# DrorT/demucs

Measured on NVIDIA B200. Metric: htdemucs audio-seconds separated per second, higher is better.
Workload: dtype f32 (bf16 hi/lo split operands, 3 tcgen05 products, fp32 accumulate)

## Files before the change

### demucs_b200/csrc/gemm_tc_impl.cuh

```cuda
#pragma once
#include <stdlib.h>
#include "gemm_epilogue.cuh"
#include "tcgen05.cuh"

enum { BD_TC_TF32 = 0, BD_TC_TF32X3 = 1, BD_TC_BF16X3 = 2, BD_TC_BF16 = 3, BD_TC_BF16D = 4 };

struct TileGeom {
  int R0, R1;
  int log2R0;
  int blocks0, blocks1;
  int cpb;
  int stride4;
};

namespace {

constexpr int TBM = 128;


struct RowInfo {
  long long obase;
  int i0;
  int rb_row;
  float e_mean, e_rstd;
  int pad0, pad1;
};

__device__ __forceinline__ float sigmoid_fast(float x) {
  const float e = bd_ex2_approx(-1.44269504088896340736f * x);
  float r;
  asm("rcp.approx.ftz.f32 %0, %1;" : "=f"(r) : "f"(1.0f + e));
  return r;
}
__device__ __forceinline__ float4 lds128(uint32_t a) {
  float4 v;
  asm volatile("ld.shared.v4.f32 {%0, %1, %2, %3}, [%4];" : "=f"(v.x), "=f"(v.y), "=f"(v.z), "=f"(v.w) : "r"(a));
  return v;
}

template <int ACT, bool E, bool RES, bool ROWB, bool CT, int WC, int RB>
__device__ __forceinline__ void epi_fast_rows(const bd_gemm_desc& d, uint32_t stage_s, uint32_t rinfo_s, int lane, int n0w,
                                              float& ssum, float& ssq) {
  constexpr int LDT = WC + 4;
  constexpr int CG = WC / 4 < 32 ? WC / 4 : 32;
  constexpr int RPI = 32 / CG;
  const int cg = lane % CG, rsub = lane / CG;
  const int n = n0w + 4 * cg;
  const bool col_ok = n < d.N;
  const int nc = col_ok ? n : 0;
  const float4 bias = d.bias ? ldg4(d.bias + nc) : make_float4(0.f, 0.f, 0.f, 0.f);
  float4 gam = make_float4(1.f, 1.f, 1.f, 1.f), bet = make_float4(0.f, 0.f, 0.f, 0.f);
  if (E) {
    gam = ldg4(d.e_gamma + nc);
    bet = ldg4(d.e_beta + nc);
  }
  const int no = ACT == BD_ACT_GLU ? nc >> 1 : nc;
  float4 scl = make_float4(1.f, 1.f, 1.f, 1.f);
  if (RES && d.scale) {
    if (ACT == BD_ACT_GLU) {
      const float2 t = ldg2(d.scale + no);
      scl.x = t.x; scl.y = t.y;
    } else {
      scl = ldg4(d.scale + no);
    }
  }
  int rr = 0;
  long long colofs = no;
  if (CT) {
    const int cout = d.N >> 2;
    rr = nc / cout;
    colofs = (long long)rr * d.os_0 + (nc - rr * cout);
    rr -= d.convt == 1 ? 2 : 0;
  }
  const long long outo = colofs;
  const float* resp = RES ? d.resid + colofs : nullptr;
  const float* addp = CT && d.addend ? d.addend + colofs : nullptr;
  const float* rbp = ROWB ? d.rowbias + no : nullptr;
  const int rb_ld = ACT == BD_ACT_GLU ? d.N >> 1 : d.N;
  const uint32_t st_lane = stage_s + (uint32_t)(rsub * LDT + 4 * cg) * 4u;
  const uint32_t ri_lane = rinfo_s + (uint32_t)rsub * 32u;
#pragma unroll 1
  for (int it = 0; it < 32 / RPI; it += RB) {
    long long ob[RB];
    bool ok[RB];
    float mean[RB], rstd[RB];
    float4 res[RB];
#pragma unroll
    for (int u = 0; u < RB; ++u) {
      const uint32_t ra = ri_lane + (uint32_t)((it + u) * RPI) * 32u;
      uint32_t w0, w1, w2, w3;
      asm volatile("ld.shared.v4.u32 {%0, %1, %2, %3}, [%4];" : "=r"(w0), "=r"(w1), "=r"(w2), "=r"(w3) : "r"(ra));
      ob[u] = (long long)(((unsigned long long)w1 << 32) | w0);
      ok[u] = (int)w2 >= 0 && col_ok;
      if (CT) ok[u] = ok[u] && (unsigned)(4 * (int)w2 + rr) < (unsigned)d.O0;
      if (ROWB || CT) res[u] = make_float4(0.f, 0.f, 0.f, 0.f);
      if (ROWB && ok[u]) {
        if (ACT == BD_ACT_GLU) {
          const float2 t = ldg2(rbp + (size_t)w3 * rb_ld);
          res[u].x = t.x; res[u].y = t.y;
        } else {
          res[u] = ldg4(rbp + (size_t)w3 * rb_ld);
        }
      }
      if (CT && addp && ok[u]) res[u] = ldg4(addp + ob[u]);
      if (E) asm volatile("ld.shared.v2.f32 {%0, %1}, [%2];" : "=f"(mean[u]), "=f"(rstd[u]) : "r"(ra + 16));
      if (RES) {
        res[u] = make_float4(0.f, 0.f, 0.f, 0.f);
        if (ok[u]) {
          if (ACT == BD_ACT_GLU) {
            const float2 t = ldg2(resp + ob[u]);
            res[u].x = t.x; res[u].y = t.y;
          } else {
            res[u] = ldg4(resp + ob[u]);
          }
        }
      }
    }
#pragma unroll
    for (int u = 0; u < RB; ++u) {
      float4 v = lds128(st_lane + (uint32_t)((it + u) * RPI * LDT) * 4u);
      v.x += bias.x; v.y += bias.y; v.z += bias.z; v.w += bias.w;
      if (E) {
        v.x = fmaf((v.x - mean[u]) * rstd[u], gam.x, bet.x);
        v.y = fmaf((v.y - mean[u]) * rstd[u], gam.y, bet.y);
        v.z = fmaf((v.z - mean[u]) * rstd[u], gam.z, bet.z);
        v.w = fmaf((v.w - mean[u]) * rstd[u], gam.w, bet.w);
      }
      if (ACT == BD_ACT_GLU) {
        float2 o2 = make_float2(v.x * sigmoid_fast(v.y), v.z * sigmoid_fast(v.w));
        if (ROWB) {
          o2.x += res[u].x;
          o2.y += res[u].y;
        }
        if (RES) {
          o2.x = fmaf(scl.x, o2.x, res[u].x);
          o2.y = fmaf(scl.y, o2.y, res[u].y);
        }
        if (ok[u]) {
          bd_store_out2(d, outo + ob[u], o2);
          ssum += o2.x + o2.y;
          ssq = fmaf(o2.x, o2.x, fmaf(o2.y, o2.y, ssq));
        }
      } else {
        if (ACT == BD_ACT_GELU) {
          v.x = bd_gelu(v.x); v.y = bd_gelu(v.y); v.z = bd_gelu(v.z); v.w = bd_gelu(v.w);
        }
        if (RES) {
          v.x = fmaf(scl.x, v.x, res[u].x); v.y = fmaf(scl.y, v.y, res[u].y);
          v.z = fmaf(scl.z, v.z, res[u].z); v.w = fmaf(scl.w, v.w, res[u].w);
        }
        if (ROWB || CT) {
          v.x += res[u].x; v.y += res[u].y; v.z += res[u].z; v.w += res[u].w;
        }
        if (ok[u]) {
          bd_store_out4(d, outo + ob[u], v);
          ssum += (v.x + v.y) + (v.z + v.w);
          ssq = fmaf(v.x, v.x, fmaf(v.y, v.y, fmaf(v.z, v.z, fmaf(v.w, v.w, ssq))));
        }
      }
    }
  }
}

__device__ __forceinline__ int epi_fast_id(const bd_gemm_desc& d, bool vec, bool row_stats) {
  if (!vec || row_stats || !d.out || d.oc_split) return -1;
  const bool e = d.e_stats != nullptr, r = d.resid != nullptr;
  if (d.convt) return (d.act == BD_ACT_GELU && !e && !r && !d.rowbias) ? 6 : -1;
  if (d.addend) return -1;
  if (d.rowbias) return (d.act == BD_ACT_GLU && !e && !r) ? 5 : -1;
  if (d.act == BD_ACT_NONE && !e) return r ? 1 : 0;
  if (d.act == BD_ACT_GELU && !e && !r) return 2;
  if (d.act == BD_ACT_GLU && !e && !r) return 3;
  if (d.act == BD_ACT_GLU && e && r) return 4;
  return -1;
}

#ifndef BD_TC_EPI_GROUPS
#define BD_TC_EPI_GROUPS 4
#endif
__host__ __device__ constexpr int pow2_at_least(int v, int p) { return p >= v ? p : pow2_at_least(v, 2 * p); }

template <int TBK, int TBN, int MODE, bool ATM = false>
struct PCfg {
  static_assert(!ATM || (MODE == BD_TC_BF16X3 && TBN <= 192), "A in tensor memory: strict mode, tiles up to 192 wide");
  static_assert(TBN % 16 == 0 && TBN <= 256, "UMMA N (M = 128): a multiple of 16 up to 256");
  static constexpr bool kX3 = MODE == BD_TC_TF32X3;
  static constexpr bool kB16 = MODE == BD_TC_BF16X3 || MODE == BD_TC_BF16 || MODE == BD_TC_BF16D;
  static constexpr bool kDirect = MODE == BD_TC_BF16D;
  static constexpr bool kSplit = MODE != BD_TC_TF32 && !kDirect;
  static constexpr int kBParts = MODE == BD_TC_BF16X3 ? 2 : 1;
  static constexpr int kPGroups = (MODE == BD_TC_TF32X3 || MODE == BD_TC_BF16X3) ? 2 : BD_TC_EPI_GROUPS;
  static constexpr int kSplitWarp0 = kB16 ? 2 : 4;
  static constexpr int kSplitWarps = MODE == BD_TC_BF16 ? 2 : 4;
  static constexpr int kEpiWarp0 = kSplit ? kSplitWarp0 + kSplitWarps : 4;
  static constexpr int kThreads = 32 * kEpiWarp0 + 128 * kPGroups;
  static constexpr int kTileBytesA = TBM * TBK * (kDirect ? 2 : 4);
  static constexpr int kTileBytesB = kB16 ? TBN * TBK * 2 : TBN * TBK * 4;
  static constexpr int kStageBytesA = (kX3 ? 2 : 1) * kTileBytesA;
  static constexpr int kStageBytesB = (kX3 ? 2 : kBParts) * kTileBytesB;
  static constexpr int kTxBytes = kTileBytesA + (kB16 ? kBParts : 1) * kTileBytesB;
  static constexpr bool kTileSplit = TBN <= 32;
  static constexpr int kNAcc = kTileSplit ? kPGroups : 2;
  static constexpr int kChunk = TBN == 256 ? 128 : TBN == 192 ? 64 : TBN == 96 ? 32 : TBN;
  static constexpr int kChunks = TBN / kChunk;
  static constexpr int kWarpCols = kTileSplit ? TBN : kChunk / kPGroups;
  static_assert(kWarpCols >= 16 && (kWarpCols & (kWarpCols - 1)) == 0, "epilogue: power-of-two warp column range");
  static constexpr int kStagingBytes = 4 * kPGroups * 32 * (kWarpCols + 4) * 4;
  static constexpr int kTailBytes = 512 + 128 * kPGroups * 32;
  static constexpr int kBudget = 227 * 1024 - 1024 - kTailBytes - kStagingBytes;
  static constexpr int kStagesRaw = kBudget / (kStageBytesA + kStageBytesB);
  static constexpr int kStages = kStagesRaw > (kTileSplit ? 16 : 8) ? (kTileSplit ? 16 : 8) : kStagesRaw;
  static constexpr int kSmemBytes = kStages * (kStageBytesA + kStageBytesB) + kStagingBytes + 1024 + kTailBytes;
  static constexpr int kACol0 = kNAcc * TBN;
  static constexpr int kTmemUsed = kNAcc * TBN + (ATM ? kStages * TBK : 0);
  static_assert(kTmemUsed <= 512, "tensor memory: accumulators + A ring exceed 512 columns");
  static constexpr int kTmemCols = pow2_at_least(kTmemUsed, 32);
};

template <int TBK, int TBN, int MODE, bool ATM>
__global__ void __launch_bounds__((PCfg<TBK, TBN, MODE, ATM>::kThreads), 1) conv_gemm_tc_persist_kernel(const __grid_constant__ CUtensorMap map_a,
                                                                            const __grid_constant__ CUtensorMap map_b,
                                                                            const __grid_constant__ CUtensorMap map_b_lo,
                                                                            const bd_gemm_desc d, const TileGeom g,
                                                                            int ntiles, int ntn) {
  using C_ = PCfg<TBK, TBN, MODE, ATM>;
  constexpr bool X3 = C_::kX3, B16 = C_::kB16, SPLIT = C_::kSplit;
  constexpr int kPGroups = C_::kPGroups;
  constexpr int kTileBytesA = C_::kTileBytesA, kTileBytesB = C_::kTileBytesB;
  constexpr int kStages = C_::kStages, kStageBytesA = C_::kStageBytesA, kStageBytesB = C_::kStageBytesB;
  constexpr int kTmemCols = C_::kTmemCols;
  constexpr int WC = C_::kWarpCols;
  constexpr int CW = WC < 32 ? WC : 32;
  extern __shared__ uint8_t smem_raw[];
  uint8_t* smem = reinterpret_cast<uint8_t*>(((uintptr_t)smem_raw + 1023) & ~(uintptr_t)1023);
  uint8_t* sA = smem;
  uint8_t* sB = smem + kStages * kStageBytesA;
  float* staging = reinterpret_cast<float*>(sB + kStages * kStageBytesB);
  uint64_t* full_bar = reinterpret_cast<uint64_t*>(reinterpret_cast<uint8_t*>(staging) + C_::kStagingBytes);
  uint64_t* empty_bar = full_bar + kStages;
  constexpr int kNAcc = C_::kNAcc;
  constexpr bool kTileSplit = C_::kTileSplit;
  constexpr int NCH = C_::kChunks, CHW = C_::kChunk;
  uint64_t* tmem_full = empty_bar + kStages;
  uint64_t* tmem_empty = tmem_full + kNAcc;
  uint64_t* conv_bar = tmem_empty + kNAcc;
  uint32_t* tmem_slot = reinterpret_cast<uint32_t*>(conv_bar + kStages);

  const int warp = threadIdx.x >> 5, lane = threadIdx.x & 31;
  const int nkb = d.taps * g.cpb;

  if (threadIdx.x == 0) {
    for (int s = 0; s < kStages; ++s) {
      mbar_init(&full_bar[s], 1);
      mbar_init(&empty_bar[s], 1);
      mbar_init(&conv_bar[s], 32 * C_::kSplitWarps);
    }
    for (int a = 0; a < kNAcc; ++a) {
      mbar_init(&tmem_full[a], 1);
      mbar_init(&tmem_empty[a], kTileSplit ? 4 : 4 * kPGroups);
    }
    mbar_fence_init();
  }
  if (warp == 1) {
    tcgen05_alloc(tmem_slot, kTmemCols);
    tcgen05_relinquish();
  }
  tcgen05_fence_before();
  __syncthreads();
  tcgen05_fence_after();
  const uint32_t tmem_base = *tmem_slot;

  auto decode = [&](int tile, int& b, int& i0s, int& i1s, int& n0) {
    const int nb = tile % ntn;
    int r = tile / ntn;
    const int blk0 = r % g.blocks0;
    r /= g.blocks0;
    const int blk1 = r % g.blocks1;
    b = r / g.blocks1;
    i0s = blk0 * g.R0;
    i1s = blk1 * g.R1;
    n0 = nb * TBN;
  };

  if (warp == 0) {
    if (lane == 0) {
      long long kbg = 0;
      for (int tile = blockIdx.x; tile < ntiles; tile += gridDim.x) {
        int b, i0s, i1s, n0;
        decode(tile, b, i0s, i1s, n0);
        int tap = 0, cb = 0;
        for (int kb = 0; kb < nkb; ++kb, ++kbg) {
          const int s = (int)(kbg % kStages);
          const uint32_t ph = (uint32_t)((kbg / kStages) & 1);
          mbar_wait_parked(&empty_bar[s], ph ^ 1);
          mbar_expect_tx(&full_bar[s], C_::kTxBytes);
          if (g.stride4) {
            const int d0 = d.d0[tap];
            tma_load_5d(&map_a, &full_bar[s], sA + s * kStageBytesA, cb * TBK, d0 & 3, i0s + (d0 >> 2), i1s + d.d1[tap], b);
          } else {
            tma_load_4d(&map_a, &full_bar[s], sA + s * kStageBytesA, cb * TBK, i0s + d.d0[tap], i1s + d.d1[tap], b);
          }
          tma_load_2d(&map_b, &full_bar[s], sB + s * kStageBytesB, tap * d.Cin + cb * TBK, n0);
          if constexpr (MODE == BD_TC_BF16X3)
            tma_load_2d(&map_b_lo, &full_bar[s], sB + s * kStageBytesB + kTileBytesB, tap * d.Cin + cb * TBK, n0);
          if (++cb == g.cpb) {
            cb = 0;
            ++tap;
// ... 99 lines not shown
      constexpr int RB = TBK * 4, RH = TBK * 2;
      constexpr int GB = 8 * RB;
      constexpr int SW = C_::kSplitWarps;
      constexpr int NG = (TBM / 8) / SW;
      const int sw = warp - C_::kSplitWarp0, r = lane >> 2, q = lane & 3;
      const int xin = (r * RB >> 7) & (RB / 16 - 1);
      const int xout = (r * RH >> 7) & (RH / 16 - 1);
      (void)et;
      for (int tile = blockIdx.x; tile < ntiles; tile += gridDim.x) {
        for (int kb = 0; kb < nkb; ++kb, ++kbg) {
          const int s = (int)(kbg % kStages);
          mbar_wait(&full_bar[s], (uint32_t)((kbg / kStages) & 1));
          uint8_t* base = sA + s * kStageBytesA;
#pragma unroll
          for (int i0 = 0; i0 < NG; i0 += 4) {
          float4 v[4][TBK == 32 ? 2 : 1];
#pragma unroll
          for (int i = 0; i < 4; ++i) {
            const uint8_t* gp = base + (sw + SW * (i0 + i)) * GB + r * RB;
            if constexpr (TBK == 32) {
              v[i][0] = *reinterpret_cast<const float4*>(gp + (((2 * q) ^ xin) << 4));
              v[i][1] = *reinterpret_cast<const float4*>(gp + (((2 * q + 1) ^ xin) << 4));
            } else {
              v[i][0] = *reinterpret_cast<const float4*>(gp + ((q ^ xin) << 4));
            }
          }
          __syncwarp();
#pragma unroll
          for (int i = 0; i < 4; ++i) {
            uint8_t* gp = base + (sw + SW * (i0 + i)) * GB + r * RH;
            uint32_t hi[TBK == 32 ? 4 : 2], lo[TBK == 32 ? 4 : 2];
#pragma unroll
            for (int j = 0; j < (TBK == 32 ? 2 : 1); ++j) {
              const float4 x = v[i][j];
              const uint32_t h0 = bd_pack_bf16(x.x, x.y), h1 = bd_pack_bf16(x.z, x.w);
              hi[2 * j] = h0;
              hi[2 * j + 1] = h1;
              lo[2 * j] = lo[2 * j + 1] = 0u;
              if constexpr (MODE == BD_TC_BF16X3) {
                lo[2 * j] = bd_pack_bf16(x.x - __uint_as_float(h0 << 16), x.y - __uint_as_float(h0 & 0xffff0000u));
                lo[2 * j + 1] = bd_pack_bf16(x.z - __uint_as_float(h1 << 16), x.w - __uint_as_float(h1 & 0xffff0000u));
              }
            }
            if constexpr (TBK == 32) {
              uint8_t* dst = gp + ((q ^ xout) << 4);
              *reinterpret_cast<uint4*>(dst) = make_uint4(hi[0], hi[1], hi[2], hi[3]);
              if constexpr (MODE == BD_TC_BF16X3) *reinterpret_cast<uint4*>(dst + 8 * RH) = make_uint4(lo[0], lo[1], lo[2], lo[3]);
            } else {
              uint8_t* dst = gp + (((q >> 1) ^ xout) << 4) + ((q & 1) << 3);
              *reinterpret_cast<uint2*>(dst) = make_uint2(hi[0], hi[1]);
              if constexpr (MODE == BD_TC_BF16X3) *reinterpret_cast<uint2*>(dst + 8 * RH) = make_uint2(lo[0], lo[1]);
            }
          }
          }
          asm volatile("fence.proxy.async.shared::cta;" ::: "memory");
          mbar_arrive(&conv_bar[s]);
        }
      }
    } else {
    for (int tile = blockIdx.x; tile < ntiles; tile += gridDim.x) {
      for (int kb = 0; kb < nkb; ++kb, ++kbg) {
        const int s = (int)(kbg % kStages);
        mbar_wait(&full_bar[s], (uint32_t)((kbg / kStages) & 1));
        auto split = [&](uint8_t* base, int tile_bytes) {
          float4* hi = reinterpret_cast<float4*>(base);
          float4* lo = reinterpret_cast<float4*>(base + tile_bytes);
#pragma unroll 4
          for (int i = et; i < tile_bytes / 16; i += 128) {
            const float4 x = hi[i];
            const float4 h = make_float4(bd_tf32_rna(x.x), bd_tf32_rna(x.y), bd_tf32_rna(x.z), bd_tf32_rna(x.w));
            hi[i] = h;
            lo[i] = make_float4(x.x - h.x, x.y - h.y, x.z - h.z, x.w - h.w);
          }
        };
        split(sA + s * kStageBytesA, kTileBytesA);
        split(sB + s * kStageBytesB, kTileBytesB);
        asm volatile("fence.proxy.async.shared::cta;" ::: "memory");
        mbar_arrive(&conv_bar[s]);
      }
    }
    }
  } else if (warp >= C_::kEpiWarp0) {
    const int quarter = warp & 3, ew = warp - C_::kEpiWarp0, grp = ew >> 2;
    const int cbase = kTileSplit ? 0 : grp * WC;
    const bool row_stats = d.stats_out && d.stat_mod != 1;
    const bool vec = bd_epi_vec_ok(d);
    const int fast = epi_fast_id(d, vec, row_stats);
    constexpr int LDT = WC + 4;
    float* stage = staging + (size_t)ew * 32 * LDT;
    RowInfo* rinfo = reinterpret_cast<RowInfo*>(((uintptr_t)(tmem_slot + 4) + 31) & ~(uintptr_t)31) + ew * 32;
    int tcount = 0;
    for (int tile = blockIdx.x; tile < ntiles; tile += gridDim.x, ++tcount) {
      if (kTileSplit && tcount % kPGroups != grp) continue;
      int b, i0s, i1s, n0;
      decode(tile, b, i0s, i1s, n0);
      const int a = tcount % kNAcc;
      const int r = quarter * 32 + lane;
      const int i0 = i0s + (r & (g.R0 - 1)), i1 = i1s + (r >> g.log2R0);
      const bool row_ok = i0 < d.I0 && i1 < d.I1;
      const long long m = ((long long)b * d.I1 + i1) * d.I0 + i0;
      EpiRow er;
      er.obase = 0; er.i0 = 0; er.rb_row = 0; er.e_mean = 0.f; er.e_rstd = 1.f;
      if (row_ok) {
        er.i0 = i0;
        er.obase = (long long)b * d.os_b + (long long)i1 * d.os_1 +
                   (long long)(d.convt ? 4 * i0 - (d.convt == 1 ? 2 : 0) : i0) * d.os_0;
        if (d.rowbias) er.rb_row = (int)((unsigned)m % (unsigned)d.rowbias_period);
        if (d.e_stats) {
          const int sl = bd_stat_slab(d, m);
          er.e_mean = __ldg(d.e_stats + 2 * (size_t)sl);
          er.e_rstd = __ldg(d.e_stats + 2 * (size_t)sl + 1);
        }
      }
      const int my_slab = (d.stats_out && row_ok) ? bd_stat_slab(d, m) : -1;
      float ssum = 0.f, ssq = 0.f;
      if (d.resid && row_ok && !d.convt && !d.oc_split) {
        const int c0 = n0 + cbase;
        if (c0 < d.N) {
          const float* pf = d.resid + er.obase + (d.act == BD_ACT_GLU ? c0 >> 1 : c0);
          asm volatile("prefetch.global.L2 [%0];" ::"l"(pf));
        }
      }
#pragma unroll 1
      for (int ch = 0; ch < NCH; ++ch) {
      const int n0h = n0 + CHW * ch;
      if (ch == 0) {
        mbar_wait_relaxed(&tmem_full[a], (uint32_t)((tcount / kNAcc) & 1));
        tcgen05_fence_after();
      } else {
        __syncwarp();
      }
      const bool last_chunk = ch == NCH - 1;
      const uint32_t acc = tmem_base + (uint32_t)(a * TBN + CHW * ch + cbase) + ((uint32_t)(quarter * 32) << 16);
      if (vec) {
        rinfo[lane].obase = er.obase;
        rinfo[lane].i0 = row_ok ? er.i0 : -1;
        rinfo[lane].rb_row = er.rb_row;
        rinfo[lane].e_mean = er.e_mean;
        rinfo[lane].e_rstd = er.e_rstd;
        for (int c0 = 0; c0 < WC; c0 += CW) {
          if (n0h + cbase + c0 >= d.N) break;
          uint32_t v[CW];
          if constexpr (CW == 32) tmem_ld32(acc + c0, v); else tmem_ld16(acc + c0, v);
#pragma unroll
          for (int j = 0; j < CW; j += 4)
            *reinterpret_cast<float4*>(stage + lane * LDT + c0 + j) =
                make_float4(__uint_as_float(v[j]), __uint_as_float(v[j + 1]), __uint_as_float(v[j + 2]),
                            __uint_as_float(v[j + 3]));
        }
        tcgen05_fence_before();
        __syncwarp();
        if (lane == 0 && last_chunk) mbar_arrive(&tmem_empty[a]);
        if (fast >= 0) {
          const uint32_t st_s = smem_u32(stage), ri_s = smem_u32(rinfo);
          const int n0w = n0h + cbase;
          constexpr int FRB = kPGroups >= 4 ? 2 : 4;
          switch (fast) {
            case 0: epi_fast_rows<BD_ACT_NONE, false, false, false, false, WC, FRB>(d, st_s, ri_s, lane, n0w, ssum, ssq); break;
            case 1: epi_fast_rows<BD_ACT_NONE, false, true, false, false, WC, FRB>(d, st_s, ri_s, lane, n0w, ssum, ssq); break;
            case 2: epi_fast_rows<BD_ACT_GELU, false, false, false, false, WC, FRB>(d, st_s, ri_s, lane, n0w, ssum, ssq); break;
            case 3: epi_fast_rows<BD_ACT_GLU, false, false, false, false, WC, FRB>(d, st_s, ri_s, lane, n0w, ssum, ssq); break;
            case 4: epi_fast_rows<BD_ACT_GLU, true, true, false, false, WC, FRB>(d, st_s, ri_s, lane, n0w, ssum, ssq); break;
            case 5: epi_fast_rows<BD_ACT_GLU, false, false, true, false, WC, FRB>(d, st_s, ri_s, lane, n0w, ssum, ssq); break;
            default: epi_fast_rows<BD_ACT_GELU, false, false, false, true, WC, FRB>(d, st_s, ri_s, lane, n0w, ssum, ssq); break;
          }
          __syncwarp();
        } else {
        constexpr int CG = WC / 4 < 32 ? WC / 4 : 32;
        constexpr int RPI = 32 / CG;
        constexpr int RB = kPGroups >= 4 ? 2 : 4;
        const int cg = lane % CG, rsub = lane / CG;
        const int n = n0h + cbase + 4 * cg;
        const bool col_ok = n < d.N;
        EpiCol ecol;
        if (col_ok) ecol = bd_epi_cols4(d, n);
        for (int it = 0; it < 32 / RPI; it += RB) {
          EpiRow row[RB];
          EpiMem mem[RB];
          bool ok[RB];
#pragma unroll
          for (int u = 0; u < RB; ++u) {
            const int rloc = (it + u) * RPI + rsub;
            const uint32_t ra = smem_u32(&rinfo[rloc]);
            uint32_t w0, w1, w2, w3, w4, w5;
            asm volatile("ld.shared.v4.u32 {%0, %1, %2, %3}, [%4];" : "=r"(w0), "=r"(w1), "=r"(w2), "=r"(w3) : "r"(ra));
            asm volatile("ld.shared.v2.u32 {%0, %1}, [%2];" : "=r"(w4), "=r"(w5) : "r"(ra + 16));
            row[u].obase = (long long)(((unsigned long long)w1 << 32) | w0);
            row[u].i0 = (int)w2;
            row[u].rb_row = (int)w3;
            row[u].e_mean = __uint_as_float(w4);
            row[u].e_rstd = __uint_as_float(w5);
            ok[u] = row[u].i0 >= 0 && col_ok;
            if (ok[u]) mem[u] = bd_epi_fetch4(d, row[u], ecol);
          }
#pragma unroll
          for (int u = 0; u < RB; ++u) {
            const int rloc = (it + u) * RPI + rsub;
            float rs = 0.f, rq = 0.f;
            if (ok[u]) {
              const float4 acc4 = *reinterpret_cast<const float4*>(stage + rloc * LDT + 4 * cg);
              bd_epi_finish4(d, row[u], ecol, acc4, mem[u], rs, rq);
            }
            if (row_stats) {
              __syncwarp();
              *reinterpret_cast<float2*>(stage + rloc * LDT + 2 * cg) = make_float2(rs, rq);
            } else {
              ssum += rs;
              ssq += rq;
            }
          }
        }
        if (row_stats) {
          __syncwarp();
          float rs = 0.f, rq = 0.f;
#pragma unroll
          for (int c = 0; c < CG; ++c) {
            const float2 t = *reinterpret_cast<const float2*>(stage + lane * LDT + 2 * c);
            rs += t.x;
            rq += t.y;
          }
          if (my_slab >= 0) {
            atomicAdd(&d.stats_out[2 * (size_t)my_slab], (double)rs);
            atomicAdd(&d.stats_out[2 * (size_t)my_slab + 1], (double)rq);
          }
        }
        __syncwarp();
        }
      } else {
        for (int c0 = 0; c0 < WC; c0 += CW) {
          if (n0h + cbase + c0 >= d.N) break;
          uint32_t v[CW];
          if constexpr (CW == 32) tmem_ld32(acc + c0, v); else tmem_ld16(acc + c0, v);
          if (row_ok) {
#pragma unroll
            for (int j = 0; j < CW; ++j) {
              const int n = n0h + cbase + c0 + j;
              if (n < d.N) {
                float st;
                if (bd_epi_apply(d, er, n, __uint_as_float(v[j]), __uint_as_float(v[(j + 1) % CW]), st)) {
                  ssum += st;
                  ssq = fmaf(st, st, ssq);
                }
              }
            }
          }
        }
        tcgen05_fence_before();
        __syncwarp();
        if (lane == 0 && last_chunk) mbar_arrive(&tmem_empty[a]);
      }
      }
      if (!vec && row_stats && row_ok) {
        atomicAdd(&d.stats_out[2 * (size_t)my_slab], (double)ssum);
        atomicAdd(&d.stats_out[2 * (size_t)my_slab + 1], (double)ssq);
      }
      if (d.stats_out && d.stat_mod == 1) {
        const double ds = bd_warp_sum_d((double)ssum), dq = bd_warp_sum_d((double)ssq);
        if (lane == 0) {
          const int sl = bd_stat_slab(d, (long long)b * d.I1 * d.I0 + i0s);
          atomicAdd(&d.stats_out[2 * (size_t)sl], ds);
          atomicAdd(&d.stats_out[2 * (size_t)sl + 1], dq);
        }
      }
    }
  }
  tcgen05_fence_before();
  __syncthreads();
  if (warp == 1) {
    tcgen05_fence_after();
    tcgen05_dealloc(tmem_base, kTmemCols);
  }
}

template <int TBK, int TBN, int MODE, bool ATM = false>
int launch_tc_persist(const bd_gemm_desc& d, const TileGeom& g, int items, cudaStream_t st) {
  using C_ = PCfg<TBK, TBN, MODE, ATM>;
  alignas(64) CUtensorMap map_a, map_b, map_b_lo;
  const long long s0 = d.xs_0, s1 = d.J1 > 1 ? d.xs_1 : s0 * d.J0, sb = items > 1 ? d.xs_b : s1 * d.J1;
  constexpr int ES = C_::kDirect ? 2 : 4;
  cuuint64_t adim[5] = {(cuuint64_t)d.Cin, (cuuint64_t)d.J0, (cuuint64_t)d.J1, (cuuint64_t)items, 1};
  cuuint64_t astr[4] = {(cuuint64_t)s0 * ES, (cuuint64_t)s1 * ES, (cuuint64_t)sb * ES, 0};
  cuuint32_t abox[5] = {(cuuint32_t)TBK, (cuuint32_t)g.R0, (cuuint32_t)g.R1, 1, 1};
  int arank = 4;
  if (g.stride4) {
    arank = 5;
    adim[1] = 4; adim[2] = (cuuint64_t)d.J0 / 4; adim[3] = (cuuint64_t)d.J1; adim[4] = (cuuint64_t)items;
    astr[0] = (cuuint64_t)s0 * ES; astr[1] = (cuuint64_t)s0 * 4 * ES; astr[2] = (cuuint64_t)s1 * ES; astr[3] = (cuuint64_t)sb * ES;
    abox[1] = 1; abox[2] = (cuuint32_t)g.R0; abox[3] = (cuuint32_t)g.R1; abox[4] = 1;
  }
  cuuint64_t bdim[2] = {(cuuint64_t)d.K, (cuuint64_t)d.N};
  cuuint32_t bbox[2] = {(cuuint32_t)TBK, (cuuint32_t)TBN};
  bool ok = encode_tensor_map(&map_a, d.x, arank, adim, astr, abox, TBK * ES, C_::kDirect);
  if constexpr (C_::kB16) {
    cuuint64_t bstr[1] = {(cuuint64_t)d.K * 2};
    ok = ok && encode_tensor_map(&map_b, d.w16_hi, 2, bdim, bstr, bbox, TBK * 2, true);
    ok = ok && encode_tensor_map(&map_b_lo, MODE == BD_TC_BF16X3 ? d.w16_lo : d.w16_hi, 2, bdim, bstr, bbox, TBK * 2, true);
  } else {
    cuuint64_t bstr[1] = {(cuuint64_t)d.K * 4};
    ok = ok && encode_tensor_map(&map_b, d.w, 2, bdim, bstr, bbox, TBK * 4);
    map_b_lo = map_b;
  }
  if (!ok) {
    bd_set_error("bd_conv_gemm_tc: TMA tensor map encoding failed (M=%d N=%d K=%d Cin=%d J0=%d J1=%d)", d.M, d.N, d.K,
                 d.Cin, d.J0, d.J1);
    return BD_ERR_CUDA;
  }
  static int sms_of[64] = {0};
  int dev = 0;
  cudaGetDevice(&dev);
  if (dev < 0 || dev >= 64) {
    bd_set_error("bd_conv_gemm_tc: device ordinal %d out of range", dev);
    return BD_ERR_ARG;
  }
  if (!sms_of[dev]) {
    cudaError_t e = cudaFuncSetAttribute(conv_gemm_tc_persist_kernel<TBK, TBN, MODE, ATM>,
                                         cudaFuncAttributeMaxDynamicSharedMemorySize, C_::kSmemBytes);
    if (e != cudaSuccess) {
      bd_set_error("bd_conv_gemm_tc: cudaFuncSetAttribute: %s", cudaGetErrorString(e));
      return BD_ERR_CUDA;
    }
    int n = 0;
    cudaDeviceGetAttribute(&n, cudaDevAttrMultiProcessorCount, dev);
    sms_of[dev] = n;
  }
  const int sms = sms_of[dev];
  const int ntn = (d.N + TBN - 1) / TBN;
  const long long ntiles = (long long)items * g.blocks1 * g.blocks0 * ntn;
  const int grid = (int)(ntiles < sms ? ntiles : sms);
  conv_gemm_tc_persist_kernel<TBK, TBN, MODE, ATM><<<grid, C_::kThreads, C_::kSmemBytes, st>>>(map_a, map_b, map_b_lo, d,
                                                                                              g, (int)ntiles, ntn);
  return bd_check_launch("conv_gemm_tc_persist_kernel");
}

template <int TBK, int MODE, bool ATM = false>
int launch_tc_width(int tbn, const bd_gemm_desc& d, const TileGeom& g, int items, cudaStream_t st) {
  switch (tbn) {
    case 16: return launch_tc_persist<TBK, 16, MODE, ATM>(d, g, items, st);
    case 32: return launch_tc_persist<TBK, 32, MODE, ATM>(d, g, items, st);
    case 64: return launch_tc_persist<TBK, 64, MODE, ATM>(d, g, items, st);
    case 128: return launch_tc_persist<TBK, 128, MODE, ATM>(d, g, items, st);
    default: break;
  }
  if constexpr (MODE == BD_TC_BF16X3) {
    if (tbn == 96) return launch_tc_persist<TBK, 96, MODE, ATM>(d, g, items, st);
    if (tbn == 192) return launch_tc_persist<TBK, 192, MODE, ATM>(d, g, items, st);
  }
  bd_set_error("bd_conv_gemm_tc: no kernel for tile width %d", tbn);
  return BD_ERR_ARG;
}

}
```

### demucs_b200/csrc/tcgen05.cuh

```cuda
#pragma once
#include <cuda.h>
#include "common.cuh"

namespace {

constexpr uint32_t kSpinLimit = 1u << 26;

__device__ __forceinline__ uint32_t smem_u32(const void* p) { return (uint32_t)__cvta_generic_to_shared(p); }

__device__ __forceinline__ void mbar_init(uint64_t* bar, uint32_t count) {
  asm volatile("mbarrier.init.shared::cta.b64 [%0], %1;" ::"r"(smem_u32(bar)), "r"(count));
}
__device__ __forceinline__ void mbar_fence_init() { asm volatile("fence.mbarrier_init.release.cluster;" ::: "memory"); }
__device__ __forceinline__ void mbar_arrive(uint64_t* bar) {
  asm volatile("mbarrier.arrive.shared::cta.b64 _, [%0];" ::"r"(smem_u32(bar)) : "memory");
}
__device__ __forceinline__ void mbar_expect_tx(uint64_t* bar, uint32_t bytes) {
  asm volatile("mbarrier.arrive.expect_tx.shared::cta.b64 _, [%0], %1;" ::"r"(smem_u32(bar)), "r"(bytes) : "memory");
}
__device__ __forceinline__ void mbar_wait(uint64_t* bar, uint32_t parity) {
  uint32_t done = 0, spins = 0;
  while (true) {
    asm volatile(
        "{\n\t.reg .pred p;\n\t"
        "mbarrier.try_wait.parity.shared::cta.b64 p, [%1], %2;\n\t"
        "selp.u32 %0, 1, 0, p;\n\t}"
        : "=r"(done)
        : "r"(smem_u32(bar)), "r"(parity)
        : "memory");
    if (done) return;
    if (++spins > kSpinLimit) __trap();
  }
}
__device__ __forceinline__ void mbar_wait_parked(uint64_t* bar, uint32_t parity) {
  uint32_t done = 0, spins = 0;
  while (true) {
    asm volatile(
        "{\n\t.reg .pred p;\n\t"
        "mbarrier.try_wait.parity.shared::cta.b64 p, [%1], %2, %3;\n\t"
        "selp.u32 %0, 1, 0, p;\n\t}"
        : "=r"(done)
        : "r"(smem_u32(bar)), "r"(parity), "r"(1000)
        : "memory");
    if (done) return;
    if (++spins > kSpinLimit) __trap();
  }
}
__device__ __forceinline__ void mbar_wait_relaxed(uint64_t* bar, uint32_t parity) {
  uint32_t done = 0, spins = 0;
  while (true) {
    asm volatile(
        "{\n\t.reg .pred p;\n\t"
        "mbarrier.try_wait.parity.shared::cta.b64 p, [%1], %2;\n\t"
        "selp.u32 %0, 1, 0, p;\n\t}"
        : "=r"(done)
        : "r"(smem_u32(bar)), "r"(parity)
        : "memory");
    if (done) return;
    __nanosleep(64);
    if (++spins > kSpinLimit) __trap();
  }
}

__device__ __forceinline__ void tma_load_2d(const CUtensorMap* map, uint64_t* bar, void* dst, int c0, int c1) {
  asm volatile(
      "cp.async.bulk.tensor.2d.shared::cluster.global.mbarrier::complete_tx::bytes [%0], [%1, {%3, %4}], [%2];"
      ::"r"(smem_u32(dst)), "l"((uint64_t)map), "r"(smem_u32(bar)), "r"(c0), "r"(c1)
      : "memory");
}
__device__ __forceinline__ void tma_load_3d(const CUtensorMap* map, uint64_t* bar, void* dst, int c0, int c1, int c2) {
  asm volatile(
      "cp.async.bulk.tensor.3d.shared::cluster.global.mbarrier::complete_tx::bytes [%0], [%1, {%3, %4, %5}], [%2];"
      ::"r"(smem_u32(dst)), "l"((uint64_t)map), "r"(smem_u32(bar)), "r"(c0), "r"(c1), "r"(c2)
      : "memory");
}
__device__ __forceinline__ void tma_load_4d(const CUtensorMap* map, uint64_t* bar, void* dst, int c0, int c1, int c2,
                                            int c3) {
  asm volatile(
      "cp.async.bulk.tensor.4d.shared::cluster.global.mbarrier::complete_tx::bytes [%0], [%1, {%3, %4, %5, %6}], [%2];"
      ::"r"(smem_u32(dst)), "l"((uint64_t)map), "r"(smem_u32(bar)), "r"(c0), "r"(c1), "r"(c2), "r"(c3)
      : "memory");
}
__device__ __forceinline__ void tma_load_5d(const CUtensorMap* map, uint64_t* bar, void* dst, int c0, int c1, int c2,
                                            int c3, int c4) {
  asm volatile(
      "cp.async.bulk.tensor.5d.shared::cluster.global.mbarrier::complete_tx::bytes [%0], [%1, {%3, %4, %5, %6, %7}], "
      "[%2];"
      ::"r"(smem_u32(dst)), "l"((uint64_t)map), "r"(smem_u32(bar)), "r"(c0), "r"(c1), "r"(c2), "r"(c3), "r"(c4)
      : "memory");
}

__device__ __forceinline__ void tcgen05_alloc(uint32_t* slot, uint32_t cols) {
  asm volatile("tcgen05.alloc.cta_group::1.sync.aligned.shared::cta.b32 [%0], %1;" ::"r"(smem_u32(slot)), "r"(cols));
}
__device__ __forceinline__ void tcgen05_relinquish() {
  asm volatile("tcgen05.relinquish_alloc_permit.cta_group::1.sync.aligned;" ::);
}
__device__ __forceinline__ void tcgen05_dealloc(uint32_t base, uint32_t cols) {
  asm volatile("tcgen05.dealloc.cta_group::1.sync.aligned.b32 %0, %1;" ::"r"(base), "r"(cols));
}
__device__ __forceinline__ void tcgen05_commit(uint64_t* bar) {
  asm volatile("tcgen05.commit.cta_group::1.mbarrier::arrive::one.shared::cluster.b64 [%0];" ::"r"(smem_u32(bar))
               : "memory");
}
__device__ __forceinline__ void tcgen05_fence_after() { asm volatile("tcgen05.fence::after_thread_sync;" ::: "memory"); }
__device__ __forceinline__ void tcgen05_fence_before() { asm volatile("tcgen05.fence::before_thread_sync;" ::: "memory"); }

__device__ __forceinline__ void umma_tf32(uint32_t tmem_d, uint64_t adesc, uint64_t bdesc, uint32_t idesc, uint32_t accumulate) {
  asm volatile(
      "{\n\t.reg .pred p;\n\t"
      "setp.ne.b32 p, %4, 0;\n\t"
      "tcgen05.mma.cta_group::1.kind::tf32 [%0], %1, %2, %3, p;\n\t}"
      ::"r"(tmem_d), "l"(adesc), "l"(bdesc), "r"(idesc), "r"(accumulate)
      : "memory");
}
__device__ __forceinline__ void umma_tf32_ts(uint32_t tmem_d, uint32_t tmem_a, uint64_t bdesc, uint32_t idesc, uint32_t accumulate) {
  asm volatile(
      "{\n\t.reg .pred p;\n\t"
      "setp.ne.b32 p, %4, 0;\n\t"
      "tcgen05.mma.cta_group::1.kind::tf32 [%0], [%1], %2, %3, p;\n\t}"
      ::"r"(tmem_d), "r"(tmem_a), "l"(bdesc), "r"(idesc), "r"(accumulate)
      : "memory");
}
__device__ __forceinline__ void umma_bf16(uint32_t tmem_d, uint64_t adesc, uint64_t bdesc, uint32_t idesc, uint32_t accumulate) {
  asm volatile(
      "{\n\t.reg .pred p;\n\t"
      "setp.ne.b32 p, %4, 0;\n\t"
      "tcgen05.mma.cta_group::1.kind::f16 [%0], %1, %2, %3, p;\n\t}"
      ::"r"(tmem_d), "l"(adesc), "l"(bdesc), "r"(idesc), "r"(accumulate)
      : "memory");
}
__device__ __forceinline__ void umma_bf16_ts(uint32_t tmem_d, uint32_t tmem_a, uint64_t bdesc, uint32_t idesc, uint32_t accumulate) {
  asm volatile(
      "{\n\t.reg .pred p;\n\t"
      "setp.ne.b32 p, %4, 0;\n\t"
      "tcgen05.mma.cta_group::1.kind::f16 [%0], [%1], %2, %3, p;\n\t}"
      ::"r"(tmem_d), "r"(tmem_a), "l"(bdesc), "r"(idesc), "r"(accumulate)
      : "memory");
}

__device__ __forceinline__ uint64_t smem_desc(const void* smem, int sbo, int layout) {
  uint64_t desc = (uint64_t)((smem_u32(smem) & 0x3FFFF) >> 4);
  desc |= (uint64_t)(sbo >> 4) << 32;
  desc |= (uint64_t)1 << 46;
  desc |= (uint64_t)layout << 61;
  return desc;
}
__device__ __forceinline__ uint64_t desc_sw128(const void* smem) { return smem_desc(smem, 1024, 2); }
template <int TBK>
__device__ __forceinline__ uint64_t make_kmajor_desc(const void* smem) {
  return smem_desc(smem, 8 * TBK * 4, TBK == 32 ? 2 : 4);
}
template <int TBK>
__device__ __forceinline__ uint64_t make_kmajor_desc16(const void* smem, int sbo) {
  return smem_desc(smem, sbo, TBK == 64 ? 2 : TBK == 32 ? 4 : 6);
}
__host__ __device__ constexpr uint32_t make_idesc_tf32(int M, int N, int b_mn_major = 0) {
  return (1u << 4) | (2u << 7) | (2u << 10) | ((uint32_t)b_mn_major << 16) | ((uint32_t)(N >> 3) << 17) |
         ((uint32_t)(M >> 4) << 24);
}
__host__ __device__ constexpr uint32_t make_idesc_bf16(int M, int N, int b_mn_major = 0) {
  return (1u << 4) | (1u << 7) | (1u << 10) | ((uint32_t)b_mn_major << 16) | ((uint32_t)(N >> 3) << 17) |
         ((uint32_t)(M >> 4) << 24);
}

__device__ __forceinline__ void tmem_ld_wait() { asm volatile("tcgen05.wait::ld.sync.aligned;" ::: "memory"); }
__device__ __forceinline__ void tmem_st_wait() { asm volatile("tcgen05.wait::st.sync.aligned;" ::: "memory"); }
__device__ __forceinline__ void tmem_ld32_nowait(uint32_t taddr, uint32_t* r) {
  asm volatile(
      "tcgen05.ld.sync.aligned.32x32b.x32.b32 "
      "{%0, %1, %2, %3, %4, %5, %6, %7, %8, %9, %10, %11, %12, %13, %14, %15, "
      "%16, %17, %18, %19, %20, %21, %22, %23, %24, %25, %26, %27, %28, %29, %30, %31}, [%32];"
      : "=r"(r[0]), "=r"(r[1]), "=r"(r[2]), "=r"(r[3]), "=r"(r[4]), "=r"(r[5]), "=r"(r[6]), "=r"(r[7]), "=r"(r[8]),
        "=r"(r[9]), "=r"(r[10]), "=r"(r[11]), "=r"(r[12]), "=r"(r[13]), "=r"(r[14]), "=r"(r[15]), "=r"(r[16]),
        "=r"(r[17]), "=r"(r[18]), "=r"(r[19]), "=r"(r[20]), "=r"(r[21]), "=r"(r[22]), "=r"(r[23]), "=r"(r[24]),
        "=r"(r[25]), "=r"(r[26]), "=r"(r[27]), "=r"(r[28]), "=r"(r[29]), "=r"(r[30]), "=r"(r[31])
      : "r"(taddr));
}
__device__ __forceinline__ void tmem_ld32(uint32_t taddr, uint32_t* r) {
  tmem_ld32_nowait(taddr, r);
  tmem_ld_wait();
}
__device__ __forceinline__ void tmem_ld16(uint32_t taddr, uint32_t* r) {
  asm volatile(
      "tcgen05.ld.sync.aligned.32x32b.x16.b32 "
      "{%0, %1, %2, %3, %4, %5, %6, %7, %8, %9, %10, %11, %12, %13, %14, %15}, [%16];"
      : "=r"(r[0]), "=r"(r[1]), "=r"(r[2]), "=r"(r[3]), "=r"(r[4]), "=r"(r[5]), "=r"(r[6]), "=r"(r[7]), "=r"(r[8]),
        "=r"(r[9]), "=r"(r[10]), "=r"(r[11]), "=r"(r[12]), "=r"(r[13]), "=r"(r[14]), "=r"(r[15])
      : "r"(taddr));
  tmem_ld_wait();
}
__device__ __forceinline__ void tmem_st32(uint32_t taddr, const uint32_t* r) {
  asm volatile(
      "tcgen05.st.sync.aligned.32x32b.x32.b32 [%0], "
      "{%1, %2, %3, %4, %5, %6, %7, %8, %9, %10, %11, %12, %13, %14, %15, %16, "
      "%17, %18, %19, %20, %21, %22, %23, %24, %25, %26, %27, %28, %29, %30, %31, %32};"
      ::"r"(taddr), "r"(r[0]), "r"(r[1]), "r"(r[2]), "r"(r[3]), "r"(r[4]), "r"(r[5]), "r"(r[6]), "r"(r[7]), "r"(r[8]),
        "r"(r[9]), "r"(r[10]), "r"(r[11]), "r"(r[12]), "r"(r[13]), "r"(r[14]), "r"(r[15]), "r"(r[16]), "r"(r[17]),
        "r"(r[18]), "r"(r[19]), "r"(r[20]), "r"(r[21]), "r"(r[22]), "r"(r[23]), "r"(r[24]), "r"(r[25]), "r"(r[26]),
        "r"(r[27]), "r"(r[28]), "r"(r[29]), "r"(r[30]), "r"(r[31])
      : "memory");
}
__device__ __forceinline__ void tmem_st16(uint32_t taddr, const uint32_t* r) {
  asm volatile(
      "tcgen05.st.sync.aligned.32x32b.x16.b32 [%0], "
      "{%1, %2, %3, %4, %5, %6, %7, %8, %9, %10, %11, %12, %13, %14, %15, %16};"
      ::"r"(taddr), "r"(r[0]), "r"(r[1]), "r"(r[2]), "r"(r[3]), "r"(r[4]), "r"(r[5]), "r"(r[6]), "r"(r[7]), "r"(r[8]),
        "r"(r[9]), "r"(r[10]), "r"(r[11]), "r"(r[12]), "r"(r[13]), "r"(r[14]), "r"(r[15])
      : "memory");
}

typedef CUresult (*EncodeTiledFn)(CUtensorMap*, CUtensorMapDataType, cuuint32_t, void*, const cuuint64_t*,
                                  const cuuint64_t*, const cuuint32_t*, const cuuint32_t*, CUtensorMapInterleave,
                                  CUtensorMapSwizzle, CUtensorMapL2promotion, CUtensorMapFloatOOBfill);

EncodeTiledFn get_encode_fn() {
  static EncodeTiledFn fn = nullptr;
  if (!fn) {
    void* p = nullptr;
    cudaDriverEntryPointQueryResult q;
    if (cudaGetDriverEntryPoint("cuTensorMapEncodeTiled", &p, cudaEnableDefault, &q) != cudaSuccess ||
        q != cudaDriverEntryPointSuccess)
      return nullptr;
    fn = (EncodeTiledFn)p;
  }
  return fn;
}

bool encode_tensor_map(CUtensorMap* map, const void* base, int rank, const cuuint64_t* gdim,
                       const cuuint64_t* gstride_bytes, const cuuint32_t* box, int row_bytes, bool bf16 = false) {
  EncodeTiledFn enc = get_encode_fn();
  if (!enc) return false;
  cuuint32_t estr[5] = {1, 1, 1, 1, 1};
  const CUtensorMapSwizzle sw = row_bytes == 128 ? CU_TENSOR_MAP_SWIZZLE_128B
                                : row_bytes == 64 ? CU_TENSOR_MAP_SWIZZLE_64B : CU_TENSOR_MAP_SWIZZLE_32B;
  return enc(map, bf16 ? CU_TENSOR_MAP_DATA_TYPE_BFLOAT16 : CU_TENSOR_MAP_DATA_TYPE_FLOAT32, rank, (void*)base, gdim,
             gstride_bytes, box, estr, CU_TENSOR_MAP_INTERLEAVE_NONE, sw, CU_TENSOR_MAP_L2_PROMOTION_L2_128B,
             CU_TENSOR_MAP_FLOAT_OOB_FILL_NONE) == CUDA_SUCCESS;
}

}
```

Before: 2654.

## Store BF16X3 GEMM epilogue output through TMA bulk tensor stores

For the BF16X3 persistent tcgen05 GEMM, the epilogue now packs each warp's finished 32-row tile into shared staging and issues a 4D TMA tensor store, instead of per-thread global stores. Row statistics for the plain case are computed by warp shuffles plus double atomics keyed by a per-row slab index, so those GEMMs can also use the TMA path. The aim is to cut scattered global store instructions and free epilogue warps sooner. In exchange it adds bulk-group waits before staging is reused, a fourth tensor map per launch, and double-precision atomics for stats.

```diff
diff --git a/demucs_b200/csrc/gemm_tc_impl.cuh b/demucs_b200/csrc/gemm_tc_impl.cuh
--- a/demucs_b200/csrc/gemm_tc_impl.cuh
+++ b/demucs_b200/csrc/gemm_tc_impl.cuh
@@ -23,7 +23,8 @@
   int i0;
   int rb_row;
   float e_mean, e_rstd;
-  int pad0, pad1;
+  int slab;
+  int pad;
 };
 
 __device__ __forceinline__ float sigmoid_fast(float x) {
@@ -38,10 +39,12 @@
   return v;
 }
 
-template <int ACT, bool E, bool RES, bool ROWB, bool CT, int WC, int RB>
+template <int ACT, bool E, bool RES, bool ROWB, bool CT, int WC, int RB, bool TMA = false, bool RS = false>
 __device__ __forceinline__ void epi_fast_rows(const bd_gemm_desc& d, uint32_t stage_s, uint32_t rinfo_s, int lane, int n0w,
                                               float& ssum, float& ssq) {
+  static_assert(!RS || (TMA && ACT == BD_ACT_NONE && !E && !RES && !ROWB && !CT), "row statistics: plain TMA epilogue");
   constexpr int LDT = WC + 4;
+  constexpr int WCO = ACT == BD_ACT_GLU ? WC / 2 : WC;
   constexpr int CG = WC / 4 < 32 ? WC / 4 : 32;
   constexpr int RPI = 32 / CG;
   const int cg = lane % CG, rsub = lane / CG;
@@ -79,12 +82,16 @@
   const int rb_ld = ACT == BD_ACT_GLU ? d.N >> 1 : d.N;
   const uint32_t st_lane = stage_s + (uint32_t)(rsub * LDT + 4 * cg) * 4u;
   const uint32_t ri_lane = rinfo_s + (uint32_t)rsub * 32u;
+  const int es = d.out_bf16 ? 2 : 4;
+  const uint32_t box_lane = stage_s + (uint32_t)((rsub * WCO + (ACT == BD_ACT_GLU ? 2 : 4) * cg) * es);
 #pragma unroll 1
   for (int it = 0; it < 32 / RPI; it += RB) {
     long long ob[RB];
     bool ok[RB];
     float mean[RB], rstd[RB];
     float4 res[RB];
+    float4 acc[RB];
+    int slab[RB];
 #pragma unroll
     for (int u = 0; u < RB; ++u) {
       const uint32_t ra = ri_lane + (uint32_t)((it + u) * RPI) * 32u;
@@ -104,6 +111,7 @@
       }
       if (CT && addp && ok[u]) res[u] = ldg4(addp + ob[u]);
       if (E) asm volatile("ld.shared.v2.f32 {%0, %1}, [%2];" : "=f"(mean[u]), "=f"(rstd[u]) : "r"(ra + 16));
+      if (RS) asm volatile("ld.shared.s32 %0, [%1];" : "=r"(slab[u]) : "r"(ra + 24));
       if (RES) {
         res[u] = make_float4(0.f, 0.f, 0.f, 0.f);
         if (ok[u]) {
@@ -116,9 +124,15 @@
         }
       }
     }
+    if (TMA) {
+#pragma unroll
+      for (int u = 0; u < RB; ++u) acc[u] = lds128(st_lane + (uint32_t)((it + u) * RPI * LDT) * 4u);
+      __syncwarp();
+    }
 #pragma unroll
     for (int u = 0; u < RB; ++u) {
-      float4 v = lds128(st_lane + (uint32_t)((it + u) * RPI * LDT) * 4u);
+      float4 v = TMA ? acc[u] : lds128(st_lane + (uint32_t)((it + u) * RPI * LDT) * 4u);
+      const uint32_t bo = box_lane + (uint32_t)((it + u) * RPI * WCO * es);
       v.x += bias.x; v.y += bias.y; v.z += bias.z; v.w += bias.w;
       if (E) {
         v.x = fmaf((v.x - mean[u]) * rstd[u], gam.x, bet.x);
@@ -136,8 +150,14 @@
           o2.x = fmaf(scl.x, o2.x, res[u].x);
           o2.y = fmaf(scl.y, o2.y, res[u].y);
         }
+        if (TMA) {
+          if (d.out_bf16)
+            asm volatile("st.shared.u32 [%0], %1;" ::"r"(bo), "r"(bd_pack_bf16(o2.x, o2.y)) : "memory");
+          else
+            asm volatile("st.shared.v2.f32 [%0], {%1, %2};" ::"r"(bo), "f"(o2.x), "f"(o2.y) : "memory");
+        }
         if (ok[u]) {
-          bd_store_out2(d, outo + ob[u], o2);
+          if (!TMA) bd_store_out2(d, outo + ob[u], o2);
           ssum += o2.x + o2.y;
           ssq = fmaf(o2.x, o2.x, fmaf(o2.y, o2.y, ssq));
         }
@@ -152,8 +172,32 @@
         if (ROWB || CT) {
           v.x += res[u].x; v.y += res[u].y; v.z += res[u].z; v.w += res[u].w;
         }
-        if (ok[u]) {
-          bd_store_out4(d, outo + ob[u], v);
+        if (TMA) {
+          if (d.out_bf16)
+            asm volatile("st.shared.v2.u32 [%0], {%1, %2};" ::"r"(bo), "r"(bd_pack_bf16(v.x, v.y)), "r"(bd_pack_bf16(v.z, v.w))
+                         : "memory");
+          else
+            asm volatile("st.shared.v4.f32 [%0], {%1, %2, %3, %4};" ::"r"(bo), "f"(v.x), "f"(v.y), "f"(v.z), "f"(v.w)
+                         : "memory");
+        }
+        if (RS) {
+          float rs = 0.f, rq = 0.f;
+          if (ok[u]) {
+            rs = (v.x + v.y) + (v.z + v.w);
+            rq = fmaf(v.x, v.x, fmaf(v.y, v.y, fmaf(v.z, v.z, fmaf(v.w, v.w, 0.f))));
+          }
+          float ts = 0.f, tq = 0.f;
+#pragma unroll
+          for (int c = 0; c < CG; ++c) {
+            ts += __shfl_sync(0xffffffffu, rs, rsub * CG + c);
+            tq += __shfl_sync(0xffffffffu, rq, rsub * CG + c);
+          }
+          if (cg == 0 && slab[u] >= 0) {
+            atomicAdd(&d.stats_out[2 * (size_t)slab[u]], (double)ts);
+            atomicAdd(&d.stats_out[2 * (size_t)slab[u] + 1], (double)tq);
+          }
+        } else if (ok[u]) {
+          if (!TMA) bd_store_out4(d, outo + ob[u], v);
           ssum += (v.x + v.y) + (v.z + v.w);
           ssq = fmaf(v.x, v.x, fmaf(v.y, v.y, fmaf(v.z, v.z, fmaf(v.w, v.w, ssq))));
         }
@@ -162,7 +206,7 @@
   }
 }
 
-__device__ __forceinline__ int epi_fast_id(const bd_gemm_desc& d, bool vec, bool row_stats) {
+__host__ __device__ __forceinline__ int epi_fast_id(const bd_gemm_desc& d, bool vec, bool row_stats) {
   if (!vec || row_stats || !d.out || d.oc_split) return -1;
   const bool e = d.e_stats != nullptr, r = d.resid != nullptr;
   if (d.convt) return (d.act == BD_ACT_GELU && !e && !r && !d.rowbias) ? 6 : -1;
@@ -203,6 +247,7 @@
   static constexpr int kNAcc = kTileSplit ? kPGroups : 2;
   static constexpr int kChunk = TBN == 256 ? 128 : TBN == 192 ? 64 : TBN == 96 ? 32 : TBN;
   static constexpr int kChunks = TBN / kChunk;
+  static constexpr bool kTmaStore = MODE == BD_TC_BF16X3;
   static constexpr int kWarpCols = kTileSplit ? TBN : kChunk / kPGroups;
   static_assert(kWarpCols >= 16 && (kWarpCols & (kWarpCols - 1)) == 0, "epilogue: power-of-two warp column range");
   static constexpr int kStagingBytes = 4 * kPGroups * 32 * (kWarpCols + 4) * 4;
@@ -221,8 +266,9 @@
 __global__ void __launch_bounds__((PCfg<TBK, TBN, MODE, ATM>::kThreads), 1) conv_gemm_tc_persist_kernel(const __grid_constant__ CUtensorMap map_a,
                                                                             const __grid_constant__ CUtensorMap map_b,
                                                                             const __grid_constant__ CUtensorMap map_b_lo,
+                                                                            const __grid_constant__ CUtensorMap map_o,
                                                                             const bd_gemm_desc d, const TileGeom g,
-                                                                            int ntiles, int ntn) {
+                                                                            int ntiles, int ntn, int tma_out_arg) {
   using C_ = PCfg<TBK, TBN, MODE, ATM>;
   constexpr bool X3 = C_::kX3, B16 = C_::kB16, SPLIT = C_::kSplit;
   constexpr int kPGroups = C_::kPGroups;
@@ -488,10 +534,11 @@
     }
   } else if (warp >= C_::kEpiWarp0) {
     const int quarter = warp & 3, ew = warp - C_::kEpiWarp0, grp = ew >> 2;
+    const bool tma_out = C_::kTmaStore && tma_out_arg;
     const int cbase = kTileSplit ? 0 : grp * WC;
     const bool row_stats = d.stats_out && d.stat_mod != 1;
     const bool vec = bd_epi_vec_ok(d);
-    const int fast = epi_fast_id(d, vec, row_stats);
+    const int fast = tma_out ? epi_fast_id(d, vec, false) : epi_fast_id(d, vec, row_stats);
     constexpr int LDT = WC + 4;
     float* stage = staging + (size_t)ew * 32 * LDT;
     RowInfo* rinfo = reinterpret_cast<RowInfo*>(((uintptr_t)(tmem_slot + 4) + 31) & ~(uintptr_t)31) + ew * 32;
@@ -539,6 +586,11 @@
       const bool last_chunk = ch == NCH - 1;
       const uint32_t acc = tmem_base + (uint32_t)(a * TBN + CHW * ch + cbase) + ((uint32_t)(quarter * 32) << 16);
       if (vec) {
+        if (tma_out) {
+          if (lane == 0) bulk_wait_group_read<0>();
+          __syncwarp();
+        }
+        rinfo[lane].slab = my_slab;
         rinfo[lane].obase = er.obase;
         rinfo[lane].i0 = row_ok ? er.i0 : -1;
         rinfo[lane].rb_row = er.rb_row;
@@ -557,7 +609,30 @@
         tcgen05_fence_before();
         __syncwarp();
         if (lane == 0 && last_chunk) mbar_arrive(&tmem_empty[a]);
-        if (fast >= 0) {
+        if (tma_out) {
+          const uint32_t st_s = smem_u32(stage), ri_s = smem_u32(rinfo);
+          const int n0w = n0h + cbase;
+          constexpr int FRB = kPGroups >= 4 ? 2 : 4;
+          switch (fast) {
+            case 0:
+              if (row_stats)
+                epi_fast_rows<BD_ACT_NONE, false, false, false, false, WC, FRB, true, true>(d, st_s, ri_s, lane, n0w, ssum, ssq);
+              else
+                epi_fast_rows<BD_ACT_NONE, false, false, false, false, WC, FRB, true>(d, st_s, ri_s, lane, n0w, ssum, ssq);
+              break;
+            case 1: epi_fast_rows<BD_ACT_NONE, false, true, false, false, WC, FRB, true>(d, st_s, ri_s, lane, n0w, ssum, ssq); break;
+            case 2: epi_fast_rows<BD_ACT_GELU, false, false, false, false, WC, FRB, true>(d, st_s, ri_s, lane, n0w, ssum, ssq); break;
+            case 3: epi_fast_rows<BD_ACT_GLU, false, false, false, false, WC, FRB, true>(d, st_s, ri_s, lane, n0w, ssum, ssq); break;
+            default: epi_fast_rows<BD_ACT_GLU, true, true, false, false, WC, FRB, true>(d, st_s, ri_s, lane, n0w, ssum, ssq); break;
+          }
+          fence_proxy_async_shared();
+          __syncwarp();
+          if (lane == 0 && n0w < d.N) {
+            const int r0 = quarter * 32;
+            tma_store_4d(&map_o, stage, d.act == BD_ACT_GLU ? n0w >> 1 : n0w, i0s + (r0 & (g.R0 - 1)), i1s + (r0 >> g.log2R0), b);
+            bulk_commit_group();
+          }
+        } else if (fast >= 0) {
           const uint32_t st_s = smem_u32(stage), ri_s = smem_u32(rinfo);
           const int n0w = n0h + cbase;
           constexpr int FRB = kPGroups >= 4 ? 2 : 4;
@@ -669,6 +744,7 @@
         }
       }
     }
+    if (tma_out && lane == 0) bulk_wait_group_read<0>();
   }
   tcgen05_fence_before();
   __syncthreads();
@@ -678,10 +754,19 @@
   }
 }
 
+bool tma_store_ok(const bd_gemm_desc& d, int items) {
+  if (getenv("BD_TC_REG_STORE") != nullptr) return false;
+  const int fast = epi_fast_id(d, bd_epi_vec_ok(d), false);
+  if (fast < 0 || fast > 4) return false;
+  if (d.stats_out && d.stat_mod != 1 && fast != 0) return false;
+  const long long es = d.out_bf16 ? 2 : 4;
+  return (d.os_0 * es) % 16 == 0 && (d.I1 == 1 || (d.os_1 * es) % 16 == 0) && (items == 1 || (d.os_b * es) % 16 == 0);
+}
+
 template <int TBK, int TBN, int MODE, bool ATM = false>
 int launch_tc_persist(const bd_gemm_desc& d, const TileGeom& g, int items, cudaStream_t st) {
   using C_ = PCfg<TBK, TBN, MODE, ATM>;
-  alignas(64) CUtensorMap map_a, map_b, map_b_lo;
+  alignas(64) CUtensorMap map_a, map_b, map_b_lo, map_o;
   const long long s0 = d.xs_0, s1 = d.J1 > 1 ? d.xs_1 : s0 * d.J0, sb = items > 1 ? d.xs_b : s1 * d.J1;
   constexpr int ES = C_::kDirect ? 2 : 4;
   cuuint64_t adim[5] = {(cuuint64_t)d.Cin, (cuuint64_t)d.J0, (cuuint64_t)d.J1, (cuuint64_t)items, 1};
@@ -706,6 +791,17 @@
     ok = ok && encode_tensor_map(&map_b, d.w, 2, bdim, bstr, bbox, TBK * 4);
     map_b_lo = map_b;
   }
+  const int tma_out = C_::kTmaStore && tma_store_ok(d, items);
+  map_o = map_a;
+  if (tma_out) {
+    const int glu = d.act == BD_ACT_GLU, es = d.out_bf16 ? 2 : 4;
+    const long long o0 = d.os_0, o1 = d.I1 > 1 ? d.os_1 : o0 * d.I0, ob = items > 1 ? d.os_b : o1 * d.I1;
+    const int br0 = g.R0 < 32 ? g.R0 : 32;
+    cuuint64_t odim[4] = {(cuuint64_t)(d.N >> glu), (cuuint64_t)d.I0, (cuuint64_t)d.I1, (cuuint64_t)items};
+    cuuint64_t ostr[3] = {(cuuint64_t)(o0 * es), (cuuint64_t)(o1 * es), (cuuint64_t)(ob * es)};
+    cuuint32_t obox[4] = {(cuuint32_t)(C_::kWarpCols >> glu), (cuuint32_t)br0, (cuuint32_t)(32 / br0), 1};
+    ok = ok && encode_tensor_map(&map_o, d.out, 4, odim, ostr, obox, 0, d.out_bf16 != 0);
+  }
   if (!ok) {
     bd_set_error("bd_conv_gemm_tc: TMA tensor map encoding failed (M=%d N=%d K=%d Cin=%d J0=%d J1=%d)", d.M, d.N, d.K,
                  d.Cin, d.J0, d.J1);
@@ -733,8 +829,8 @@
   const int ntn = (d.N + TBN - 1) / TBN;
   const long long ntiles = (long long)items * g.blocks1 * g.blocks0 * ntn;
   const int grid = (int)(ntiles < sms ? ntiles : sms);
-  conv_gemm_tc_persist_kernel<TBK, TBN, MODE, ATM><<<grid, C_::kThreads, C_::kSmemBytes, st>>>(map_a, map_b, map_b_lo, d,
-                                                                                              g, (int)ntiles, ntn);
+  conv_gemm_tc_persist_kernel<TBK, TBN, MODE, ATM><<<grid, C_::kThreads, C_::kSmemBytes, st>>>(map_a, map_b, map_b_lo, map_o, d,
+                                                                                              g, (int)ntiles, ntn, tma_out);
   return bd_check_launch("conv_gemm_tc_persist_kernel");
 }
 
diff --git a/demucs_b200/csrc/tcgen05.cuh b/demucs_b200/csrc/tcgen05.cuh
--- a/demucs_b200/csrc/tcgen05.cuh
+++ b/demucs_b200/csrc/tcgen05.cuh
@@ -90,6 +90,34 @@
       : "memory");
 }
 
+__device__ __forceinline__ void tma_store_2d(const CUtensorMap* map, const void* src, int c0, int c1) {
+  asm volatile("cp.async.bulk.tensor.2d.global.shared::cta.bulk_group [%0, {%2, %3}], [%1];"
+               ::"l"((uint64_t)map), "r"(smem_u32(src)), "r"(c0), "r"(c1)
+               : "memory");
+}
+__device__ __forceinline__ void tma_store_3d(const CUtensorMap* map, const void* src, int c0, int c1, int c2) {
+  asm volatile("cp.async.bulk.tensor.3d.global.shared::cta.bulk_group [%0, {%2, %3, %4}], [%1];"
+               ::"l"((uint64_t)map), "r"(smem_u32(src)), "r"(c0), "r"(c1), "r"(c2)
+               : "memory");
+}
+__device__ __forceinline__ void tma_store_4d(const CUtensorMap* map, const void* src, int c0, int c1, int c2, int c3) {
+  asm volatile("cp.async.bulk.tensor.4d.global.shared::cta.bulk_group [%0, {%2, %3, %4, %5}], [%1];"
+               ::"l"((uint64_t)map), "r"(smem_u32(src)), "r"(c0), "r"(c1), "r"(c2), "r"(c3)
+               : "memory");
+}
+__device__ __forceinline__ void tma_store_5d(const CUtensorMap* map, const void* src, int c0, int c1, int c2, int c3,
+                                             int c4) {
+  asm volatile("cp.async.bulk.tensor.5d.global.shared::cta.bulk_group [%0, {%2, %3, %4, %5, %6}], [%1];"
+               ::"l"((uint64_t)map), "r"(smem_u32(src)), "r"(c0), "r"(c1), "r"(c2), "r"(c3), "r"(c4)
+               : "memory");
+}
+__device__ __forceinline__ void bulk_commit_group() { asm volatile("cp.async.bulk.commit_group;" ::: "memory"); }
+template <int N>
+__device__ __forceinline__ void bulk_wait_group_read() {
+  asm volatile("cp.async.bulk.wait_group.read %0;" ::"n"(N) : "memory");
+}
+__device__ __forceinline__ void fence_proxy_async_shared() { asm volatile("fence.proxy.async.shared::cta;" ::: "memory"); }
+
 __device__ __forceinline__ void tcgen05_alloc(uint32_t* slot, uint32_t cols) {
   asm volatile("tcgen05.alloc.cta_group::1.sync.aligned.shared::cta.b32 [%0], %1;" ::"r"(smem_u32(slot)), "r"(cols));
 }
@@ -233,7 +261,8 @@
   if (!enc) return false;
   cuuint32_t estr[5] = {1, 1, 1, 1, 1};
   const CUtensorMapSwizzle sw = row_bytes == 128 ? CU_TENSOR_MAP_SWIZZLE_128B
-                                : row_bytes == 64 ? CU_TENSOR_MAP_SWIZZLE_64B : CU_TENSOR_MAP_SWIZZLE_32B;
+                                : row_bytes == 64 ? CU_TENSOR_MAP_SWIZZLE_64B
+                                : row_bytes == 32 ? CU_TENSOR_MAP_SWIZZLE_32B : CU_TENSOR_MAP_SWIZZLE_NONE;
   return enc(map, bf16 ? CU_TENSOR_MAP_DATA_TYPE_BFLOAT16 : CU_TENSOR_MAP_DATA_TYPE_FLOAT32, rank, (void*)base, gdim,
              gstride_bytes, box, estr, CU_TENSOR_MAP_INTERLEAVE_NONE, sw, CU_TENSOR_MAP_L2_PROMOTION_L2_128B,
              CU_TENSOR_MAP_FLOAT_OOB_FILL_NONE) == CUDA_SUCCESS;
```

Result: no change. 2659, median of 6 (+0.2%).
